# Amandaynzhou/MMT-PSM

Hardware: AMD Instinct MI355X
Metric: imgs/sec (student+teacher step, 1000x1000, AUG_K=2) (higher is better)
Workload: dtype f32

## Files before the change

### include/mmtpsm.h

```cpp
#ifndef MMTPSM_H
#define MMTPSM_H
#include <stdint.h>
#ifdef __cplusplus
extern "C" {
#endif

#define MMT_EINVAL (-22)

int mmt_version(void);

typedef struct {
  const float* feat[4];
  float* grad_feat[4];
  int H[4];
  int W[4];
  float scale[4];
  int num_levels;
  int N;
  int C;
} mmt_pyramid;

int mmt_roi_align_forward(const mmt_pyramid* pyr , const float* rois, const int32_t* levels,
                          int K, int PH, int PW, int sampling_ratio, float* out, void* stream);
int mmt_roi_align_forward_bf16(const mmt_pyramid* pyr , const float* rois, const int32_t* levels,
// ... 120 lines not shown
  int y_amax_stats;
  const void* f16_guard_x;
  const void* f16_guard_dy;
  const void* w_src;
  const void* w_src_scale;
  int x_planes_layout;
  void* y_rb;
  long y_rb_stride;
  const float* y_rb_scale;
  void* y_amax_next;
  int x_planes_lag;
  int y_rb_rows;
} mmt_conv_args;

int mmt_conv_forward(const mmt_conv_args* a , void* stream);
int mmt_conv_variant(const mmt_conv_args* a );
int mmt_conv_ksplit(const mmt_conv_args* a );
int mmt_conv_wants_planes(const mmt_conv_args* a );
int mmt_set_conv_precision(int mode);
int mmt_amax(const float* x, long n, const float* rowscale, long inner, int rows, float* amax , void* stream);
int mmt_amax_stats(const float* x, long n, float* slot , void* stream);
int mmt_sum_stats(const float* a, const float* b, const float* c, const float* d, float* y, long n,
                  float* slot , void* stream);
int mmt_stats_combine(const float* const* slots , int n, float* out , void* stream);
int mmt_split_planes_f16(const float* x, void* planes, long plane_stride, long n, float scale, const float* amax ,
                         float* scale_out , float* amax_next ,
                         float* zero_slot , void* stream);
int mmt_pack_weight_f16(const float* w, void* planes, long plane_stride, int Cout, int K, float scale, const float* amax,
                        float* scale_out, void* stream);
int mmt_pack_weight_flipped_f16(const float* w, const float* scale, void* planes, long plane_stride, int Cout, int KH, int KW,
                                int Cin, const float* amax, float* scale_out, void* stream);
int mmt_conv3x3_strip_f16x2(const mmt_conv_args* a , const float* s_x , const float* s_w , void* stream);
int mmt_conv_forward_f16x2(const mmt_conv_args* a , const float* x_amax , const float* s_w , void* stream);
int mmt_get_conv_precision(void);
int mmt_stem_fused(const float* x, int N, int H, int W, const float* w_s2d, const void* w_planes, long w_plane_stride,
                   const float* s_w , const float* scale, const float* shift, const float* x_slot , float* y,
                   float* y_slot , void* stream);
int mmt_c64_conv3_fused(const float* x, int N, int H, int W, const float* w2, const void* w2_planes, long w2_plane_stride,
                        const float* s_w2 , const float* scale2, const float* shift2, const float* x_slot ,
                        const float* w3, const void* w3_planes, long w3_plane_stride, const float* s_w3 , const float* scale3,
                        const float* shift3, const float* res, float* out, float* out_slot ,
                        const float* o2_scale , int o2_scale_is_amax, float* o2_amax_next ,
                        float* out_amax_next , const float* w1, const void* w1_planes, long w1_plane_stride,
                        const float* s_w1 , const float* scale1, const float* shift1, const float* out_scale ,
                        float* o1_next, float* o1_next_slot , void* stream);
int mmt_conv_wgrad_planes_splits(const mmt_conv_args* a );
int mmt_conv_wgrad_planes(const mmt_conv_args* a , const float* dy, const void* x_planes, long x_plane_stride,
                          const void* dy_planes, long dy_plane_stride, const float* s_x, const float* s_dy, const float* rowscale,
                          float* dw, float* dbias, float* workspace, void* stream);
typedef struct {
  void* fn;
  long a[16];
} mmt_call;
int mmt_replay(const mmt_call* calls , int n, int* failed_index );
int mmt_split_planes_f16_rb(const float* x, void* planes, long plane_stride, int rows, int W, int C, const float* amax,
                            float* scale_out, void* stream);
int mmt_conv_writes_rb(const mmt_conv_args* a );
typedef struct mmt_wgrad_job {
  mmt_conv_args a;
  const float* dy; const float* rowscale; float* dw; float* dbias;
  const void* x_planes; long x_plane_stride; const void* dy_planes; long dy_plane_stride; const float* s_x; const float* s_dy;
} mmt_wgrad_job;
int mmt_conv_wgrad_group_workspace(const mmt_wgrad_job* jobs , int n, long* floats_out );
int mmt_conv_wgrad_group(const mmt_wgrad_job* jobs , int n, float* workspace, long workspace_floats, void* stream);
int mmt_sum_stats_rb(const float* a, const float* b, const float* c, const float* d, float* y, int rows, int W, int C, float* slot,
                     void* planes, long plane_stride, const float* scale, float* amax_next, void* stream);
// ... 143 lines not shown
```

### mmt-psm_amd/csrc/conv_igemm.hip

```cpp
#include <stdlib.h>
#include <map>
#include <mutex>
#include <type_traits>
#include "conv_shared.h"

namespace {

template <int BM, int BN, int WM, int WN>
__device__ __forceinline__ void conv_epilogue_stage(f32x16 (&acc)[BM / (32 * WM)][BN / (32 * WN)], float* lds,
                                                    const int lane, const int wm, const int wn) {
  constexpr int TM = BM / (32 * WM), TN = BN / (32 * WN);
  float* ct = lds;
  const int col_l = lane & 31, rq = lane >> 5;
#pragma unroll
  for (int a = 0; a < TM; a++)
#pragma unroll
    for (int b = 0; b < TN; b++)
#pragma unroll
      for (int r = 0; r < 16; r++) {
        const int row = (wm * TM + a) * 32 + (r & 3) + 8 * (r >> 2) + 4 * rq;
        ct[row * BN + (wn * TN + b) * 32 + col_l] = acc[a][b][r];
      }
}


__device__ __forceinline__ void conv_amax_commit(const ConvP& p, AmaxAcc a, const int lin) {
  __shared__ float red[3][8];
  const int t = threadIdx.x, w = t >> 6, nw = (blockDim.x + 63) >> 6;
  const bool stats = p.amax_stats && (lin & 63) == 0;
#pragma unroll
  for (int o = 32; o > 0; o >>= 1) a.amx = fmaxf(a.amx, __shfl_xor(a.amx, o, 64));
  if (stats) {
#pragma unroll
    for (int o = 32; o > 0; o >>= 1) { a.asum += __shfl_xor(a.asum, o, 64); a.acnt += __shfl_xor(a.acnt, o, 64); }
  }
  if ((t & 63) == 0) { red[0][w] = a.amx; red[1][w] = a.asum; red[2][w] = a.acnt; }
  __syncthreads();
  if (t == 0) {
    float m = red[0][0], sm = red[1][0], cn = red[2][0];
    for (int i = 1; i < nw; i++) { m = fmaxf(m, red[0][i]); sm += red[1][i]; cn += red[2][i]; }
    const unsigned bits = __builtin_bit_cast(unsigned, m);
    if (m > 0.f && bits > __hip_atomic_load(p.amax_out, __ATOMIC_RELAXED, __HIP_MEMORY_SCOPE_AGENT)) atomicMax(p.amax_out, bits);
    if (p.amax_next && m > 0.f && bits > __hip_atomic_load(p.amax_next, __ATOMIC_RELAXED, __HIP_MEMORY_SCOPE_AGENT)) atomicMax(p.amax_next, bits);
    if (stats && cn > 0.f) {
      const int k = (lin >> 6) & 15;
      atomicAdd((float*)p.amax_out + 1 + k, sm);
      atomicAdd((float*)p.amax_out + 17 + k, cn);
    }
  }
}

template <int BM, int BN>
__device__ __forceinline__ void conv_epilogue_finish(const ConvP& p, float* lds, const int m0, const int n0, const int tid,
                                                     const int HoWo, AmaxAcc* acc = nullptr) {
  float amx = 0.f, asum = 0.f, acnt = 0.f;
  {
    float* ct = lds;
    constexpr int C4 = BN / 4, RPP = 256 / C4;
    const int cc = tid % C4, r0 = tid / C4;
    const int c = n0 + cc * 4;
    if (c < p.Cout) {
      const bool vec = (p.Cout & 3) == 0;
      const int nv = vec ? 4 : min(4, p.Cout - c);
      float sc[4], sh[4];
#pragma unroll
      for (int e = 0; e < 4; e++) {
        sc[e] = (p.scale && e < nv) ? p.scale[c + e] : 1.f;
        sh[e] = (p.shift && e < nv) ? p.shift[c + e] : 0.f;
      }
      auto ld = [&](const float* q, float* o) {
        if (vec) { const f32x4 t = ldg4(q); o[0] = t[0]; o[1] = t[1]; o[2] = t[2]; o[3] = t[3]; }
        else { for (int e = 0; e < 4; e++) o[e] = e < nv ? q[e] : 0.f; }
      };
      auto ldh = [&](const float* base, long idx, float* o) {
        const unsigned short* q = (const unsigned short*)base + idx;
        if (vec) {
          const uint2 t = *(const uint2*)q;
          o[0] = __builtin_bit_cast(float, t.x << 16); o[1] = __builtin_bit_cast(float, t.x & 0xffff0000u);
          o[2] = __builtin_bit_cast(float, t.y << 16); o[3] = __builtin_bit_cast(float, t.y & 0xffff0000u);
        } else { for (int e = 0; e < 4; e++) o[e] = e < nv ? __builtin_bit_cast(float, (unsigned)q[e] << 16) : 0.f; }
      };
      if (p.f16_sx) {
        const float inv = 1.f / ((p.f16_ax ? f16_scale_of(*p.f16_sx) : *p.f16_sx) * *p.f16_sw);
// ... 382 lines not shown
    const char* A = ring + buf * STAGE + (wm * TM * 32) * 32 + froff;
    const char* B = ring + buf * STAGE + NS * PA + (wn * TN * 32) * 32 + froff;
    bf16x8 fa[NS][TM], fb[NS][TN];
#pragma unroll
    for (int q = 0; q < NS; q++) {
#pragma unroll
      for (int a = 0; a < TM; a++) fa[q][a] = *(const bf16x8*)(A + q * PA + a * 32 * 32);
#pragma unroll
      for (int b = 0; b < TN; b++) fb[q][b] = *(const bf16x8*)(B + q * PB + b * 32 * 32);
    }
#pragma unroll
    for (int sum = 2 * (NS - 1) > NS - 1 ? NS - 1 : 0; sum >= 0; sum--)
#pragma unroll
      for (int qa = 0; qa <= sum; qa++) {
        const int qb = sum - qa;
        if (qa < NS && qb < NS) {
#pragma unroll
          for (int a = 0; a < TM; a++)
#pragma unroll
            for (int b = 0; b < TN; b++)
              acc[a][b] = __builtin_amdgcn_mfma_f32_32x32x16_bf16(fa[qa][a], fb[qb][b], acc[a][b], 0, 0, 0);
        }
      }
    if (kt + 1 < nkt) store_tile(buf ^ 1);
    __syncthreads();
  }
  conv_epilogue<BM, BN, WM, WN>(p, acc, lds, m0, n0, tid, lane, wm, wn, HoWo);
}

__device__ __attribute__((aligned(16))) const float g_zero16[4] = {0.f, 0.f, 0.f, 0.f};

__device__ __forceinline__ void dma16(const void* g, void* l) {
  __builtin_amdgcn_global_load_lds((const __attribute__((address_space(1))) void*)g, (lds_ptr_t)l, 16, 0, 0);
}

__device__ __forceinline__ void dma16_unseen(const void* g, void* l) {
#if defined(__HIP_DEVICE_COMPILE__)
  const unsigned la = __builtin_amdgcn_readfirstlane((unsigned)(unsigned long)(__attribute__((address_space(3))) char*)l);
  asm volatile("s_mov_b32 m0, %1\n\ts_nop 0\n\tglobal_load_lds_dwordx4 %0, off" ::"v"(g), "s"(la) : "m0", "memory");
#endif
}

template <int BM, int BN, int WM, int WN, int NS, int S, bool F16 = false>
__global__ __launch_bounds__(256, 2) void conv_fwd_glds_kernel(const ConvP p, const unsigned short* __restrict__ wpl,
                                                               const long wpl_stride, const int ksplit,
                                                               float* __restrict__ ws) {
  constexpr int TM = BM / (32 * WM), TN = BN / (32 * WN);
  constexpr int A_BYTES = BM * 64;
  constexpr int PB = BN * 32;
  constexpr int STAGE = A_BYTES + NS * PB;
  constexpr int NIA = BM / 64;
  constexpr int NIB_TOT = NS * BN / 32;
  constexpr int NIB = (NIB_TOT + 3) / 4;
  constexpr int NI = NIA + NIB;
  extern __shared__ __attribute__((aligned(16))) float lds[];
  char* const ring = (char*)lds;

  const int tid = threadIdx.x;
  const int lane = tid & 63;
  const int wave = __builtin_amdgcn_readfirstlane(tid >> 6);
  const int wm = wave / WN, wn = wave % WN;

  const int tiles_m = (p.M + BM - 1) / BM;
  const int tiles_n = (p.Cout + BN - 1) / BN;
  int bid = blockIdx.x;
  {
    const int nwg = tiles_m * tiles_n * ksplit, q = nwg >> 3, r = nwg & 7, xcd = bid & 7, idx = bid >> 3;
    bid = (xcd < r ? xcd * (q + 1) : r * (q + 1) + (xcd - r) * q) + idx;
  }
  const int ks = bid % ksplit;
  bid /= ksplit;
  const int tile_m = bid / tiles_n, tile_n = bid % tiles_n;
  const int m0 = tile_m * BM, n0 = tile_n * BN;
// ... 1492 lines not shown
```

### mmt-psm_amd/csrc/conv_shared.h

```cpp
#pragma once
#include <stdlib.h>
#include <type_traits>
#include "common.h"

namespace mmtconv {

struct ConvP {
  const float* x; const float* w; const float* scale; const float* shift; const float* res;
  const float* mask; const float* mul; float* y;
  int N, H, W, Cin, Cout, KH, KW, stride, pad, Ho, Wo;
  int relu, res_mode, out_stride, out_H, out_W;
  float mask_scale;
  int M, K, cin32, cin4;
  const unsigned short* wpl; long wpl_stride;
  const unsigned short* xpl; long xpl_stride;
  unsigned short* ypl; long ypl_stride;
  unsigned* amax_out;
  int amax_stats;
  int f16_ax;
  const float* f16_sx; const float* f16_sw;
  int io;
  const float* guard_x; const float* guard_dy;
  const float* w_src; const float* w_src_scale;
  int staged_epilogue;
// ... 64 lines not shown
  for (int q = 0; q < NS; q++) {
    const unsigned a = pk_bf16(r0, r1), b = pk_bf16(r2, r3);
    o[q] = uint2{a, b};
    if (q + 1 < NS) {
      r0 -= __builtin_bit_cast(float, a << 16);
      r1 -= __builtin_bit_cast(float, a & 0xffff0000u);
      r2 -= __builtin_bit_cast(float, b << 16);
      r3 -= __builtin_bit_cast(float, b & 0xffff0000u);
    }
  }
}
__device__ __forceinline__ float f16_scale_of(const float amax) {
  if (!(amax > 0.f)) return 1.f;
  int e;
  frexpf(amax, &e);
  e = 14 - e;
  e = e > 100 ? 100 : (e < -100 ? -100 : e);
  return ldexpf(1.f, e);
}

__device__ __forceinline__ f32x4 ldg4(const float* p) { return *(const f32x4*)p; }
__device__ __forceinline__ void split4h(const f32x4 v, const float s, uint2 (&o)[2]) {
  float r[4] = {v[0] * s, v[1] * s, v[2] * s, v[3] * s};
#pragma unroll
  for (int e = 0; e < 4; e++) r[e] = fminf(fmaxf(r[e], -65504.f), 65504.f);
  _Float16 h[4], l[4];
#pragma unroll
  for (int e = 0; e < 4; e++) { h[e] = (_Float16)r[e]; l[e] = (_Float16)(r[e] - (float)h[e]); }
  o[0] = uint2{__builtin_bit_cast(unsigned, f16x2{h[0], h[1]}), __builtin_bit_cast(unsigned, f16x2{h[2], h[3]})};
  o[1] = uint2{__builtin_bit_cast(unsigned, f16x2{l[0], l[1]}), __builtin_bit_cast(unsigned, f16x2{l[2], l[3]})};
}

struct AmaxAcc { float amx = 0.f, asum = 0.f, acnt = 0.f; };

__device__ __forceinline__ unsigned rb_split1(const float v, const float s) {
  const float r = __builtin_amdgcn_fmed3f(v * s, -65504.f, 65504.f);
  const _Float16 h = (_Float16)r;
  const _Float16 l = (_Float16)(r - (float)h);
  return __builtin_bit_cast(unsigned, f16x2{h, l});
}
struct RbGeom { int Wo; float rWo; unsigned cb32; };
__device__ __forceinline__ RbGeom rb_geom(const ConvP& p) {
  return RbGeom{p.Wo, 1.f / (float)p.Wo, (unsigned)(p.Cout >> 4) * (unsigned)p.Wo * 32u};
}
__device__ __forceinline__ unsigned rb_row_off(const RbGeom& g, const int m) {
  int row = (int)(((float)m + 0.5f) * g.rWo);
  int w = m - row * g.Wo;
  if (w < 0) { row--; w += g.Wo; } else if (w >= g.Wo) { row++; w -= g.Wo; }
  return (unsigned)row * g.cb32 + (unsigned)w * 32u;
}
__device__ __forceinline__ void rb_store4(const ConvP& p, const RbGeom& g, const int m, const int c, const f32x4 v, const float s) {
  uint2 o[2];
  split4h(v, s, o);
  char* const d = (char*)p.yrb + rb_row_off(g, m) + (unsigned)(c >> 4) * ((unsigned)g.Wo * 32u) + (unsigned)(c & 15) * 2u;
  *(uint2*)d = o[0];
  *(uint2*)(d + p.yrb_stride * 2) = o[1];
}
__device__ __forceinline__ void quad_transpose(unsigned (&w)[4], const int lane) {
  const bool o1 = lane & 1, o2 = lane & 2;
#pragma unroll
  for (int pr = 0; pr < 2; pr++) {
    const unsigned send = o1 ? w[2 * pr] : w[2 * pr + 1];
    const unsigned recv = (unsigned)__builtin_amdgcn_mov_dpp((int)send, 0xB1, 0xf, 0xf, true);
    if (o1) w[2 * pr] = recv; else w[2 * pr + 1] = recv;
  }
#pragma unroll
// ... 198 lines not shown
```

### mmt-psm_amd/maskrcnn_benchmark/_hip.py

```python
import ctypes
import weakref
import os
import threading as _threading

import torch

_HERE = os.path.dirname(os.path.abspath(__file__))
LIB_PATH = os.path.join(os.path.dirname(_HERE), "libmmtpsm.so")

c_void_p, c_int, c_float, c_double, c_int64 = ctypes.c_void_p, ctypes.c_int, ctypes.c_float, ctypes.c_double, ctypes.c_int64


class Pyramid(ctypes.Structure):
    _fields_ = [("feat", c_void_p * 4), ("grad_feat", c_void_p * 4), ("H", c_int * 4), ("W", c_int * 4),
                ("scale", c_float * 4), ("num_levels", c_int), ("N", c_int), ("C", c_int)]


class RoiMaps(ctypes.Structure):
    _fields_ = [("feat", c_void_p * 4), ("grad_feat", c_void_p * 4), ("H", c_int * 4), ("W", c_int * 4), ("C", c_int * 4),
                ("c_off", c_int * 4), ("scale", c_float * 4), ("num_maps", c_int), ("N", c_int), ("out_C", c_int)]


class ConvArgs(ctypes.Structure):
    _fields_ = [("x", c_void_p), ("w", c_void_p), ("scale", c_void_p), ("shift", c_void_p), ("res", c_void_p),
# ... 102 lines not shown
                            c_void_p, c_void_p, c_void_p, c_void_p, c_void_p],
    "mmt_position_embedding": [c_void_p, c_int, c_int, c_int, c_void_p, c_void_p, c_void_p],
    "mmt_sample_fg_bg_wide": [c_void_p, c_int, c_void_p, c_void_p, c_int, c_int, c_int, c_int, c_void_p, c_void_p, c_void_p, c_void_p,
                              c_void_p],
    "mmt_rpn_loss": [c_void_p, c_void_p, c_void_p, c_void_p, c_void_p, c_void_p, ctypes.c_long, c_float, c_void_p, c_void_p, c_void_p,
                     c_void_p, c_void_p],
    "mmt_box_loss": [c_void_p, c_void_p, c_void_p, c_void_p, c_int, c_int, c_void_p, c_void_p, c_void_p, c_void_p],
    "mmt_box_loss_rows": [c_void_p, c_void_p, c_void_p, c_void_p, c_int, c_int, c_void_p, c_void_p, c_void_p, c_void_p, c_void_p],
    "mmt_relation_attention_fwd": [c_void_p, c_void_p, c_void_p, c_void_p, c_void_p, c_int, c_int, c_int, c_int, c_int, c_int, c_float,
                                   c_void_p, c_void_p, c_void_p],
    "mmt_relation_attention_bwd": [c_void_p, c_void_p, c_void_p, c_void_p, c_void_p, c_void_p, c_int, c_int, c_int, c_int, c_int, c_float,
                                   c_void_p, c_void_p, c_void_p, c_void_p, c_void_p, c_void_p],
    "mmt_ciam_fwd": [c_void_p, c_void_p, c_int, c_int, c_int, c_int, c_void_p, c_void_p, c_void_p, c_void_p, c_void_p],
    "mmt_ciam_bwd": [c_void_p, c_void_p, c_int, c_int, c_int, c_int, c_void_p, c_void_p, c_void_p, c_void_p, c_void_p, c_void_p,
                     c_void_p, c_void_p, c_void_p],
    "mmt_stats_combine": [c_void_p, c_int, c_void_p, c_void_p],
    "mmt_sum_stats": [c_void_p, c_void_p, c_void_p, c_void_p, c_void_p, ctypes.c_long, c_void_p, c_void_p],
    "mmt_split_planes_f16": [c_void_p, c_void_p, ctypes.c_long, ctypes.c_long, c_float, c_void_p, c_void_p, c_void_p, c_void_p, c_void_p],
    "mmt_split_planes_f16_rb": [c_void_p, c_void_p, ctypes.c_long, c_int, c_int, c_int, c_void_p, c_void_p, c_void_p],
    "mmt_replay": [c_void_p, c_int, c_void_p],
    "mmt_conv_writes_rb": [ctypes.POINTER(ConvArgs)],
    "mmt_conv_wgrad_group_workspace": [c_void_p, c_int, ctypes.POINTER(ctypes.c_long)],
    "mmt_conv_wgrad_group": [c_void_p, c_int, c_void_p, ctypes.c_long, c_void_p],
    "mmt_sum_stats_rb": [c_void_p, c_void_p, c_void_p, c_void_p, c_void_p, c_int, c_int, c_int, c_void_p, c_void_p, ctypes.c_long, c_void_p,
                         c_void_p, c_void_p],
    "mmt_rb_scales_update": [c_void_p, c_int, c_void_p],
    "mmt_conv_wgrad_planes_splits": [ctypes.POINTER(ConvArgs)],
    "mmt_conv_wgrad_planes": [ctypes.POINTER(ConvArgs), c_void_p, c_void_p, ctypes.c_long, c_void_p, ctypes.c_long, c_void_p, c_void_p,
                              c_void_p, c_void_p, c_void_p, c_void_p, c_void_p],
    "mmt_pack_weight_f16": [c_void_p, c_void_p, ctypes.c_long, c_int, c_int, c_float, c_void_p, c_void_p, c_void_p],
    "mmt_pack_weight_flipped_f16": [c_void_p, c_void_p, c_void_p, ctypes.c_long, c_int, c_int, c_int, c_int, c_void_p, c_void_p, c_void_p],
    "mmt_conv3x3_strip_f16x2": [ctypes.POINTER(ConvArgs), c_void_p, c_void_p, c_void_p],
    "mmt_conv_forward_f16x2": [ctypes.POINTER(ConvArgs), c_void_p, c_void_p, c_void_p],
    "mmt_conv_forward_pg": [ctypes.POINTER(ConvArgs), c_void_p, c_void_p, c_int, c_int, c_void_p],
    "mmt_conv_pg_plan": [ctypes.POINTER(ConvArgs), c_void_p, c_void_p],
    "mmt_conv_pg_wanted": [ctypes.POINTER(ConvArgs)],
    "mmt_stem_fused": [c_void_p, c_int, c_int, c_int, c_void_p, c_void_p, ctypes.c_long, c_void_p, c_void_p, c_void_p, c_void_p, c_void_p,
                       c_void_p, c_void_p],
    "mmt_c64_conv3_fused": [c_void_p, c_int, c_int, c_int, c_void_p, c_void_p, ctypes.c_long, c_void_p, c_void_p, c_void_p, c_void_p, c_void_p,
                            c_void_p, ctypes.c_long, c_void_p, c_void_p, c_void_p, c_void_p, c_void_p, c_void_p, c_void_p, c_int, c_void_p,
                            c_void_p, c_void_p, c_void_p, ctypes.c_long, c_void_p, c_void_p, c_void_p, c_void_p, c_void_p, c_void_p,
                            c_void_p],
    "mmt_maxpool3x3s2_bf16": [c_void_p, c_void_p, c_int, c_int, c_int, c_int, c_int, c_int, c_void_p],
    "mmt_gconv3x3_forward": [c_void_p, c_void_p, c_void_p, c_void_p, c_void_p, c_int, c_int, c_int, c_int, c_int, c_int, c_int, c_void_p],
    "mmt_gconv3x3_dgrad": [c_void_p, c_void_p, c_void_p, c_void_p, c_void_p, c_void_p, c_int, c_int, c_int, c_int, c_int, c_int, c_void_p],
    "mmt_gconv3x3_wgrad": [c_void_p, c_void_p, c_void_p, c_void_p, c_int, c_int, c_int, c_int, c_int, c_int, c_void_p],
    "mmt_maxpool3x3s2_backward": [c_void_p, c_void_p, c_void_p, c_int, c_int, c_int, c_int, c_void_p],
    "mmt_stem_wgrad": [c_void_p, c_void_p, c_void_p, c_void_p, c_int, c_int, c_int, c_void_p],
    "mmt_mask_bce": [c_void_p, c_void_p, c_void_p, c_int, c_int, c_int, c_float, c_void_p, c_void_p, c_void_p],
    "mmt_mgd_level_forward": [c_void_p, ctypes.POINTER(MgdTeachers), c_void_p, c_int, c_int, c_int, c_int, c_void_p, c_void_p],
    "mmt_mgd_level_backward": [c_void_p, ctypes.POINTER(MgdTeachers), c_void_p, c_int, c_int, c_int, c_int, c_void_p, c_void_p, c_void_p],
    "mmt_mgd_views_forward": [ctypes.POINTER(MgdStudents), ctypes.POINTER(MgdTeachers), c_void_p, c_int, c_int, c_int, c_int, c_void_p,
                              c_void_p],
    "mmt_mgd_views_backward": [ctypes.POINTER(MgdStudents), ctypes.POINTER(MgdTeachers), c_void_p, c_int, c_int, c_int, c_int, c_void_p,
                               c_void_p, c_void_p],
    "mmt_mask_pool": [c_void_p, c_int, c_int, c_int, c_int, c_int, c_void_p, c_void_p],
    "mmt_psm_rows": [c_void_p, c_int, c_void_p, c_int, c_int, c_void_p, c_float, c_int, c_int, c_void_p, c_void_p, c_void_p],
    "mmt_psm_variance": [c_void_p, c_int, c_int, c_int, c_int, c_void_p, c_void_p],
    "mmt_ema_update": [c_void_p, c_void_p, c_int64, c_double, c_void_p],
    "mmt_sgd_momentum": [c_void_p, c_void_p, c_void_p, c_int64, c_float, c_float, c_float, c_int, c_void_p],
    "mmt_grad_guard": [c_void_p, c_int64, c_void_p, c_void_p, c_float, c_void_p],
    "mmt_sgd_momentum_guarded": [c_void_p, c_void_p, c_void_p, c_int64, c_float, c_float, c_float, c_int, c_void_p, c_void_p],
    "mmt_paste_masks": [c_void_p, c_void_p, c_void_p, c_void_p, c_int, c_int, c_int, c_int, c_int, c_float, c_void_p, c_void_p],
    "mmt_paste_mask_stack": [c_void_p, c_void_p, c_int, c_int, c_int, c_int, c_float, c_void_p, c_void_p],
    "mmt_polygon_targets": [c_void_p, c_void_p, c_void_p, c_void_p, c_int, c_int, c_void_p, c_void_p, c_void_p],
    "mmt_mask_pack": [c_void_p, c_int, c_int, c_int, c_void_p, c_void_p, c_void_p],
# ... 422 lines not shown
    if not PG_RB:
        xp, st = f16_split(x)
        return xp, st, 0, 0
    rb = _rb_of(x)
    if rb is not None and rb[3] == "epi" and (rb[4] is None or rb[4] >= x.shape[0]):
        F16_STATS["rb_epi"] = F16_STATS.get("rb_epi", 0) + 1
        return rb[0], rb[1], 1, 1
    F16_STATS["rb_split"] = F16_STATS.get("rb_split", 0) + 1
    N, C, Hh, W = x.shape
    if x.numel() >= (1 << 30) or C % 16:
        xp, st = f16_split(x)
        return xp, st, 0, 0
    am = _amax_of(x)
    xp = torch.empty((2, x.numel()), dtype=torch.float16, device=x.device)
    st = torch.empty((1,), dtype=torch.float32, device=x.device)
    _check(lib().mmt_split_planes_f16_rb(x.data_ptr(), xp.data_ptr(), xp.stride(0), N * Hh, W, C, am[0].data_ptr(), st.data_ptr(), _stream()),
           "mmt_split_planes_f16_rb")
    _rb_attach(x, xp, st, "split")
    return xp, st, 1, 0


def _pack_f16(w, scale, flipped, pl, am):
    Cout, Cin, KH, KW = w.shape
    F16_STATS["weight_pack"] = F16_STATS.get("weight_pack", 0) + 1
    _check(lib().mmt_amax(w.data_ptr(), w.numel(), _p(scale) if flipped else None, Cin * KH * KW, Cout, am.data_ptr(), _stream()), "mmt_amax")
    if flipped:
        _check(lib().mmt_pack_weight_flipped_f16(w.data_ptr(), _p(scale), pl.data_ptr(), pl.stride(0), Cout, KH, KW, Cin,
                                                 am.data_ptr(), am.data_ptr() + 4, _stream()), "mmt_pack_weight_flipped_f16")
    else:
        _check(lib().mmt_pack_weight_f16(w.data_ptr(), pl.data_ptr(), pl.stride(0), Cout, Cin * KH * KW, 1.0, am.data_ptr(),
                                         am.data_ptr() + 4, _stream()), "mmt_pack_weight_f16")


def f16_weight_planes(w, flip_scale=None, flipped=False):
    form = "f16_dgrad" if flipped else "f16"
    flat, hit = _flat_form(w, form, flip_scale)
    if hit is not None:
        return hit
    stamp = _loose_stamp(w, flip_scale, w)
    hit = LOOSE.get(w, form, stamp, flip_scale)
    if hit is not None:
        return hit
    Cout, Cin, KH, KW = w.shape
    am = torch.zeros((2,), dtype=torch.float32, device=w.device)
    pl = torch.empty((2, packed_elems(Cin, KH * KW * Cout) if flipped else packed_elems(Cout, Cin * KH * KW)), dtype=torch.float16,
                     device=w.device)
    _pack_f16(w, flip_scale, flipped, pl, am)
    if flipped and flat is not None and flat.register(form, w, flip_scale, pl, am):
        return pl, am[1:2]
    return LOOSE.put(w, form, stamp, flip_scale, (pl, am[1:2]), w, am)


def set_bf16_storage(on):
    global _BF16_STORAGE
    if on and _DET:
        raise NotImplementedError("bf16 activation storage is not offered in deterministic mode (its kernels' summation orders were "
                                  "never examined): set_deterministic(False)")
    _BF16_STORAGE = bool(on)


def bf16_storage():
    return _BF16_STORAGE and get_conv_precision() == 1


_DET = os.environ.get("MMT_DETERMINISTIC", "0") != "0"
_DET_TORCH = None
COLSUM_MAX_BLOCKS, MASK_BCE_WS, MGD_MAX_BLOCKS, RPN_LOSS_MAX_BLOCKS, BOX_LOSS_MAX_BLOCKS = 256, 2048, 4096, 1024, 256


def _det_torch(on):
    global _DET_TORCH
    from torch.utils import deterministic as td
    if on:
        if _DET_TORCH is None:
            _DET_TORCH = (torch.are_deterministic_algorithms_enabled(), torch.is_deterministic_algorithms_warn_only_enabled(),
                          td.fill_uninitialized_memory)
        torch.use_deterministic_algorithms(True)
        td.fill_uninitialized_memory = False
    elif _DET_TORCH is not None:
        torch.use_deterministic_algorithms(_DET_TORCH[0], warn_only=_DET_TORCH[1])
        td.fill_uninitialized_memory = _DET_TORCH[2]
        _DET_TORCH = None

# ... 1042 lines not shown
    if planes_owner is not None:
        planes_owner.ensure_bf16()
    _check(lib().mmt_conv_forward(ctypes.byref(a), _stream()), "mmt_conv_forward")
    if rec:
        _profiled(a, e0, "fwd%d" % var, lib().mmt_conv_ksplit(ctypes.byref(a)), pre, ebytes)
    if y_planes is not None:
        y._mmt_planes = (y_planes, y._version)
    if amax_slot is not None:
        y._mmt_amax = (amax_slot, y._version)
    return y


def conv_forward_pg(x, w, scale=None, shift=None, stride=1, pad=0, relu=False, res=None, mask=None, mask_scale=1.0, w_shape=None,
                    f16_src=None, tile_rows=0, ksplit=0, xp=None):
    x = nhwc(x)
    N, Cin, H, W = x.shape
    src = (nhwc(w), False, None) if w is not None else (nhwc(f16_src[0]), True, f16_src[1])
    Cout, KH, KW = _weight_dims(Cin, src[0].shape if w is not None else w_shape)
    Ho, Wo = _conv_out_hw(H, W, KH, KW, stride, pad)
    a = _conv_shape(ConvArgs(), N, H, W, Cin, Cout, KH, KW, stride, pad, Ho, Wo)
    a.x = x.data_ptr()
    y = empty_nhwc(N, Cout, Ho, Wo, x.device)
    a.y = y.data_ptr()
    a.scale, a.shift, a.relu = _p(scale), _p(shift), 1 if relu else 0
    if res is not None:
        a.res, a.res_mode = nhwc(res).data_ptr(), 1
    if mask is not None:
        a.mask, a.mask_scale = nhwc(mask).data_ptr(), float(mask_scale)
    slot = _amax_slot(x.device)
    a.y_amax, a.y_amax_stats = slot.ptr, 1
    return _conv_f16(a, K_PG, x, src, y, slot, None, int(tile_rows), int(ksplit), xp, None, False)


def stem_fused(x, w_s2d, scale, shift):
    _dev(x)
    N, C, Hh, W = x.shape
    if C != 3 or not x.is_contiguous() or x.dtype != torch.float32 or (Hh & 3) or (W & 3) or tuple(w_s2d.shape) != (64, 16, 4, 4):
        raise RuntimeError("stem_fused: (N, 3, H, W) fp32 NCHW with H, W % 4 == 0 and the 64 x 16 x 4 x 4 space-to-depth filter")
    w = nhwc(w_s2d)
    am = _amax_of(x)
    if type(am[0]) is not _Slot:
        raise RuntimeError("stem_fused: the input needs a full statistics slot")
    wp16, sw = f16_weight_planes(w)
    y = empty_nhwc(N, 64, Hh // 4, W // 4, x.device)
    slot = _amax_slot(x.device)
    _check(lib().mmt_stem_fused(x.data_ptr(), N, Hh, W, w.data_ptr(), wp16.data_ptr(), wp16.stride(0), sw.data_ptr(), _p(scale), _p(shift),
                                am[0].ptr, y.data_ptr(), slot.ptr, _stream()), "mmt_stem_fused")
    y._mmt_amax = (slot, y._version)
    return y


C64_FUSE = os.environ.get("MMT_C64_FUSE", "1") != "0"


def o2_site(w3):
    return ("o2", w3.data_ptr())


def c64_fuse_enabled():
    return bool(C64_FUSE and F16X2 and RB_EPI and PROFILE is None and os.environ.get("MMT_C64") != "0" and get_conv_precision() == 3)


def out_site(w1_next):
    return ("out1", w1_next.data_ptr())


# ... 1047 lines not shown
```

### mmt-psm_amd/maskrcnn_benchmark/layers/fused.py

```python
import torch

from .. import _hip as H


_NONE = {}


def _none_like(x):
    t = _NONE.get(x.device)
    if t is None:
        t = _NONE[x.device] = torch.empty((0,), dtype=torch.float32, device=x.device)
    return t


def _dst(t):
    return getattr(t, "_flat_grad", None) if t is not None else None


def _touch(*slots):
    for d in slots:
        if d is not None:
            ent = H.GRAD_SLOTS.get(d.data_ptr())
            if ent is not None and ent[0]() is not None:
                ent[0]().touched.add(ent[1])
# ... 400 lines not shown
    @staticmethod
    def backward(ctx, g2, g3, g4, g5):
        sv = ctx.saved_tensors
        cs, inner, wi, wl = sv[0:4], sv[4:8], sv[8:12], sv[12:16]
        gs = [g2, g3, g4, g5]
        gs = [H.nhwc(g) if g is not None else torch.zeros_like(inner[k]) for k, g in enumerate(gs)]
        d_in = [None] * 4
        dwl, dbl, dwi, dbi, dcs = [None] * 4, [None] * 4, [None] * 4, [None] * 4, [None] * 4
        for k in range(4):
            d_in[k] = _dgrad(gs[k], wl[k], inner[k].shape, 1, 1, None, res=d_in[k - 1] if k > 0 else None,
                             res_mode=3 if k > 0 else 0)
            dwl[k], dbl[k] = _wgrad(inner[k], gs[k], wl[k], 1, 1, None, True, *ctx.dst[1][k])
        for k in range(4):
            dwi[k], dbi[k] = _wgrad(cs[k], d_in[k], wi[k], 1, 0, None, True, *ctx.dst[0][k])
            if ctx.needs_input_grad[k]:
                dcs[k] = _dgrad(d_in[k], wi[k], cs[k].shape, 1, 0, None, mask=cs[k], out_dtype=cs[k].dtype)
        out = list(dcs)
        for k in range(4):
            out += [dwi[k], dbi[k]]
        for k in range(4):
            out += [dwl[k], dbl[k]]
        return tuple(out) + (None, None)


class DeconvFn(torch.autograd.Function):

    @staticmethod
    def forward(ctx, x, w, b, relu, input_relu):
        x = H.nhwc(x)
        w_in = w
        w = H.nhwc(w)
        P, Cin, h, wd_ = x.shape
        Cout = w.shape[1]
        y = H.empty_nhwc(P, Cout, 2 * h, 2 * wd_, x.device)
        wf = w.permute(2, 3, 1, 0).contiguous()
        for kh in range(2):
            for kw in range(2):
                H.conv_forward(x, wf[kh, kw].view(Cout, Cin, 1, 1), None, b, relu=relu, out_stride=2,
                               out_hw=(2 * h, 2 * wd_), y_out=y, y_offset=(kh * 2 * wd_ + kw) * Cout)
        ctx.save_for_backward(x, w)
        ctx.cfgv = (input_relu, b is not None)
        ctx.dst = (_dst(w_in), _dst(b))
        return y

    @staticmethod
    def backward(ctx, g):
        x, w = ctx.saved_tensors
        input_relu, has_b = ctx.cfgv
        g = H.nhwc(g)
        dx = dw = db = None
        if ctx.needs_input_grad[1]:
            dst_w, dst_b = ctx.dst
            dw = dst_w if dst_w is not None else torch.zeros_like(w)
            H.conv_wgrad(g, x, tuple(w.shape), 2, 0, dw)
            _touch(dst_w, dst_b if has_b else None)
            if has_b:
                db = dst_b if dst_b is not None else torch.zeros((w.shape[1],), dtype=torch.float32, device=w.device)
                H.colsum(g, db)
                db = None if dst_b is not None else db
            dw = None if dst_w is not None else dw
        if ctx.needs_input_grad[0]:
            dx = H.conv_forward(g, w, stride=2, pad=0, mask=x if input_relu else None, rb_site=("dx", w.data_ptr()))
        return dx, dw, db, None, None


class RoiAlignFpnFn(torch.autograd.Function):

    @staticmethod
    def forward(ctx, rois, levels, res, scales, sr, *feats):
        feats = [H.nhwc(f) for f in feats]
        out = H.roi_align_forward(feats, scales, rois, levels, res, res, sr)
        if out.dtype == torch.float32 and H.F16X2 and H.get_conv_precision() == 3:
# ... 193 lines not shown


def relu_grad_mask(x):
    return ReluGradMaskFn.apply(x) if x.requires_grad else x


class SplitBatchFn(torch.autograd.Function):

    @staticmethod
    def forward(ctx, x, n):
        ctx.n, ctx.shape = n, x.shape
        return x[:n], x[n:]

    @staticmethod
    def backward(ctx, ga, gb):
        n, shape = ctx.n, ctx.shape
        out = H.empty_nhwc(shape[0], shape[1], shape[2], shape[3], (ga if ga is not None else gb).device)
        if ga is not None:
            out[:n].copy_(ga)
        else:
            out[:n].zero_()
        if gb is not None:
            out[n:].copy_(gb)
        else:
            out[n:].zero_()
        return out, None


def split_batch(x, n):
    return SplitBatchFn.apply(x, n)


_FORK_ON = True


_FORK_ACC = _os.environ.get("MMT_FORK_ACC", "1") != "0"


class _ForkAcc(object):
    __slots__ = ("buf", "fresh", "seen", "rb_site")

    def __init__(self, rb_site):
        self.buf, self.fresh, self.seen, self.rb_site = None, False, [], rb_site

    def put(self, t, fresh):
        first = self.buf is None
        if t is not self.buf:
            self.seen.append(t)
        self.buf, self.fresh = t, fresh
        if not fresh:
            H.drop(t)
        return first


class ForkFn(torch.autograd.Function):

    @staticmethod
    def forward(ctx, x, n, rb_site=None, acc=None):
        ctx.set_materialize_grads(False)
        ctx.rb_site = rb_site
        ctx.acc = acc
        return tuple(x.view_as(x) for _ in range(n))

    @staticmethod
    def backward(ctx, *gs):
        gs = [g for g in gs if g is not None]
# ... 78 lines not shown
```

Before: 135.4.

## Fuse 2x2 deconv forward into one f16x2 MFMA kernel launch

Adds a dedicated HIP kernel that computes all four taps of the 2x2 transposed convolution as a single GEMM over Cout*4 columns. It uses split-f16 MFMA, streams the weights into LDS through double-buffered DMA, and scatters results directly into the strided output. This replaces four separate conv_forward launches plus a per-call weight permute/contiguous copy, and reuses the activation load across all taps. Unsupported shapes or precisions fall back to the old path, and a slow scalar fallback runs when the guard flags bad inputs. Shared helpers move into conv_shared.h.

```diff
diff --git a/include/mmtpsm.h b/include/mmtpsm.h
--- a/include/mmtpsm.h
+++ b/include/mmtpsm.h
@@ -176,6 +176,7 @@
                                 int Cin, const float* amax, float* scale_out, void* stream);
 int mmt_conv3x3_strip_f16x2(const mmt_conv_args* a , const float* s_x , const float* s_w , void* stream);
 int mmt_conv_forward_f16x2(const mmt_conv_args* a , const float* x_amax , const float* s_w , void* stream);
+int mmt_deconv2x2_forward_f16x2(const mmt_conv_args* a , const float* x_amax , const float* s_w , void* stream);
 int mmt_get_conv_precision(void);
 int mmt_stem_fused(const float* x, int N, int H, int W, const float* w_s2d, const void* w_planes, long w_plane_stride,
                    const float* s_w , const float* scale, const float* shift, const float* x_slot , float* y,
diff --git a/mmt-psm_amd/csrc/conv_igemm.hip b/mmt-psm_amd/csrc/conv_igemm.hip
--- a/mmt-psm_amd/csrc/conv_igemm.hip
+++ b/mmt-psm_amd/csrc/conv_igemm.hip
@@ -23,32 +23,6 @@
       }
 }
 
-
-__device__ __forceinline__ void conv_amax_commit(const ConvP& p, AmaxAcc a, const int lin) {
-  __shared__ float red[3][8];
-  const int t = threadIdx.x, w = t >> 6, nw = (blockDim.x + 63) >> 6;
-  const bool stats = p.amax_stats && (lin & 63) == 0;
-#pragma unroll
-  for (int o = 32; o > 0; o >>= 1) a.amx = fmaxf(a.amx, __shfl_xor(a.amx, o, 64));
-  if (stats) {
-#pragma unroll
-    for (int o = 32; o > 0; o >>= 1) { a.asum += __shfl_xor(a.asum, o, 64); a.acnt += __shfl_xor(a.acnt, o, 64); }
-  }
-  if ((t & 63) == 0) { red[0][w] = a.amx; red[1][w] = a.asum; red[2][w] = a.acnt; }
-  __syncthreads();
-  if (t == 0) {
-    float m = red[0][0], sm = red[1][0], cn = red[2][0];
-    for (int i = 1; i < nw; i++) { m = fmaxf(m, red[0][i]); sm += red[1][i]; cn += red[2][i]; }
-    const unsigned bits = __builtin_bit_cast(unsigned, m);
-    if (m > 0.f && bits > __hip_atomic_load(p.amax_out, __ATOMIC_RELAXED, __HIP_MEMORY_SCOPE_AGENT)) atomicMax(p.amax_out, bits);
-    if (p.amax_next && m > 0.f && bits > __hip_atomic_load(p.amax_next, __ATOMIC_RELAXED, __HIP_MEMORY_SCOPE_AGENT)) atomicMax(p.amax_next, bits);
-    if (stats && cn > 0.f) {
-      const int k = (lin >> 6) & 15;
-      atomicAdd((float*)p.amax_out + 1 + k, sm);
-      atomicAdd((float*)p.amax_out + 17 + k, cn);
-    }
-  }
-}
 
 template <int BM, int BN>
 __device__ __forceinline__ void conv_epilogue_finish(const ConvP& p, float* lds, const int m0, const int n0, const int tid,
@@ -497,13 +471,6 @@
 
 __device__ __forceinline__ void dma16(const void* g, void* l) {
   __builtin_amdgcn_global_load_lds((const __attribute__((address_space(1))) void*)g, (lds_ptr_t)l, 16, 0, 0);
-}
-
-__device__ __forceinline__ void dma16_unseen(const void* g, void* l) {
-#if defined(__HIP_DEVICE_COMPILE__)
-  const unsigned la = __builtin_amdgcn_readfirstlane((unsigned)(unsigned long)(__attribute__((address_space(3))) char*)l);
-  asm volatile("s_mov_b32 m0, %1\n\ts_nop 0\n\tglobal_load_lds_dwordx4 %0, off" ::"v"(g), "s"(la) : "m0", "memory");
-#endif
 }
 
 template <int BM, int BN, int WM, int WN, int NS, int S, bool F16 = false>
diff --git a/mmt-psm_amd/csrc/conv_shared.h b/mmt-psm_amd/csrc/conv_shared.h
--- a/mmt-psm_amd/csrc/conv_shared.h
+++ b/mmt-psm_amd/csrc/conv_shared.h
@@ -120,6 +120,39 @@
 }
 
 struct AmaxAcc { float amx = 0.f, asum = 0.f, acnt = 0.f; };
+
+__device__ __forceinline__ void conv_amax_commit(const ConvP& p, AmaxAcc a, const int lin) {
+  __shared__ float red[3][8];
+  const int t = threadIdx.x, w = t >> 6, nw = (blockDim.x + 63) >> 6;
+  const bool stats = p.amax_stats && (lin & 63) == 0;
+#pragma unroll
+  for (int o = 32; o > 0; o >>= 1) a.amx = fmaxf(a.amx, __shfl_xor(a.amx, o, 64));
+  if (stats) {
+#pragma unroll
+    for (int o = 32; o > 0; o >>= 1) { a.asum += __shfl_xor(a.asum, o, 64); a.acnt += __shfl_xor(a.acnt, o, 64); }
+  }
+  if ((t & 63) == 0) { red[0][w] = a.amx; red[1][w] = a.asum; red[2][w] = a.acnt; }
+  __syncthreads();
+  if (t == 0) {
+    float m = red[0][0], sm = red[1][0], cn = red[2][0];
+    for (int i = 1; i < nw; i++) { m = fmaxf(m, red[0][i]); sm += red[1][i]; cn += red[2][i]; }
+    const unsigned bits = __builtin_bit_cast(unsigned, m);
+    if (m > 0.f && bits > __hip_atomic_load(p.amax_out, __ATOMIC_RELAXED, __HIP_MEMORY_SCOPE_AGENT)) atomicMax(p.amax_out, bits);
+    if (p.amax_next && m > 0.f && bits > __hip_atomic_load(p.amax_next, __ATOMIC_RELAXED, __HIP_MEMORY_SCOPE_AGENT)) atomicMax(p.amax_next, bits);
+    if (stats && cn > 0.f) {
+      const int k = (lin >> 6) & 15;
+      atomicAdd((float*)p.amax_out + 1 + k, sm);
+      atomicAdd((float*)p.amax_out + 17 + k, cn);
+    }
+  }
+}
+
+__device__ __forceinline__ void dma16_unseen(const void* g, void* l) {
+#if defined(__HIP_DEVICE_COMPILE__)
+  const unsigned la = __builtin_amdgcn_readfirstlane((unsigned)(unsigned long)(__attribute__((address_space(3))) char*)l);
+  asm volatile("s_mov_b32 m0, %1\n\ts_nop 0\n\tglobal_load_lds_dwordx4 %0, off" ::"v"(g), "s"(la) : "m0", "memory");
+#endif
+}
 
 __device__ __forceinline__ unsigned rb_split1(const float v, const float s) {
   const float r = __builtin_amdgcn_fmed3f(v * s, -65504.f, 65504.f);
diff --git a/mmt-psm_amd/csrc/deconv.hip b/mmt-psm_amd/csrc/deconv.hip
--- /dev/null
+++ b/mmt-psm_amd/csrc/deconv.hip
@@ -0,0 +1,222 @@
+#include <atomic>
+#include "conv_shared.h"
+
+namespace {
+
+__device__ __noinline__ void deconv_slow_block(const ConvPK pk, const int m0, const int n_lo, const int n_hi, const int lin) {
+  const int C = pk->Cout >> 2, HW = pk->H * pk->W, ncols = n_hi - n_lo;
+  float amx = 0.f, asum = 0.f, acnt = 0.f;
+  for (int o = threadIdx.x; o < 128 * ncols; o += blockDim.x) {
+    const int i = o / ncols, n = n_lo + (o - i * ncols);
+    const int m = m0 + i;
+    if (m >= pk->M) break;
+    const int img = m / HW, rem = m - img * HW;
+    const int h = rem / pk->W, w = rem - h * pk->W;
+    const float* xr = pk->x + (long)m * pk->Cin;
+    const float* wr = pk->w_src + n;
+    float acc = 0.f;
+    for (int ci = 0; ci < pk->Cin; ci++) acc = fmaf(xr[ci], wr[(long)ci * pk->Cout], acc);
+    const int tap = n / C, co = n - tap * C;
+    float v = acc + (pk->shift ? pk->shift[co] : 0.f);
+    if (pk->relu) v = fmaxf(v, 0.f);
+    pk->y[(((long)img * pk->out_H + 2 * h + (tap >> 1)) * pk->out_W + 2 * w + (tap & 1)) * C + co] = v;
+    const float av = fabsf(v);
+    amx = fmaxf(amx, av); asum += av; acnt += 1.f;
+  }
+  if (pk->amax_out) {
+    if (amx > 0.f) atomicMax(pk->amax_out, __builtin_bit_cast(unsigned, amx));
+    if (pk->amax_stats && (lin & 63) == 0 && acnt > 0.f) {
+      const int k = (lin >> 6) & 15;
+      atomicAdd((float*)pk->amax_out + 1 + k, asum);
+      atomicAdd((float*)pk->amax_out + 17 + k, acnt);
+    }
+  }
+}
+
+template <int KT>
+__global__ __launch_bounds__(256, 2) void deconv2x2_rows_kernel(const ConvP p, const unsigned short* __restrict__ wpl,
+                                                                const long wpl_stride, const int ppb) {
+  constexpr int NS = 2, BN = 32;
+  constexpr int PIECES = KT * NS;
+  constexpr int BBUF = PIECES * 1024;
+  constexpr unsigned OOB = 0x80000000u;
+  static_assert(PIECES % 4 == 0, "pieces per wave");
+  extern __shared__ __attribute__((aligned(16))) float lds[];
+  char* const bring = (char*)lds;
+  unsigned* const rowb = (unsigned*)(bring + 2 * BBUF);
+  float* const shl = (float*)(bring + 2 * BBUF + 512);
+  const int tid = threadIdx.x, lane = tid & 63;
+  const int wave = __builtin_amdgcn_readfirstlane(tid >> 6);
+  const int lr = lane & 31, kh2 = lane >> 5;
+  const int m0 = blockIdx.x * 128;
+  const int K = 16 * KT;
+  const int C = p.Cout >> 2;
+  const int nb32 = p.Cout >> 5, ptap = C >> 5;
+  const int nt_lo = blockIdx.y * ppb, nt_hi = min(nb32, nt_lo + ppb);
+  const int cnt = nt_hi - nt_lo;
+  if (cnt <= 0) return;
+  const F16Guard guard = f16_guard_load(p.guard_x);
+  auto issue_b = [&](int nt, int buf) {
+#pragma unroll
+    for (int i = 0; i < PIECES / 4; i++) {
+      const int piece = wave + 4 * i;
+      const int kt = piece / NS, q = piece % NS;
+      dma16_unseen(wpl + q * wpl_stride + ((long)kt * nb32 + nt) * 512 + lane * 8, bring + buf * BBUF + piece * 1024);
+    }
+  };
+  const int rot = blockIdx.x % cnt;
+  auto pn = [&](int i) {
+    int t = i + rot;
+    if (t >= cnt) t -= cnt;
+    return nt_lo + t;
+  };
+  issue_b(pn(0), 0);
+  if (f16_guard_bad(guard)) {
+    asm volatile("s_waitcnt vmcnt(0)" ::: "memory");
+    deconv_slow_block(kernarg_convp(), m0, nt_lo * BN, nt_hi * BN, blockIdx.x + gridDim.x * blockIdx.y);
+    return;
+  }
+  if (tid < 128) {
+    const int m = m0 + tid;
+    unsigned b = OOB;
+    if (m < p.M) {
+      const int HW = p.H * p.W;
+      const int img = m / HW, rem = m - img * HW;
+      const int h = rem / p.W, w = rem - h * p.W;
+      b = (unsigned)((img * p.out_H + 2 * h) * p.out_W + 2 * w) * ((unsigned)C * 4u);
+    }
+    rowb[tid] = b;
+  }
+  for (int c = tid; c < C; c += 256) shl[c] = p.shift ? p.shift[c] : 0.f;
+  uint4 fa[KT][NS];
+  const float sx = f16_scale_of(*p.f16_sx);
+  const float finv = 1.f / (sx * *p.f16_sw);
+  const int boff = lr * 32 + (((kh2 ^ (lr >> 3)) & 1) << 4);
+  const int col_l = lane & 31, rq = lane >> 5;
+  const __amdgpu_buffer_rsrc_t ry = __builtin_amdgcn_make_buffer_rsrc((void*)p.y, 0, (int)((long)p.M * p.Cout * 4), 0x00020000);
+  {
+    const __amdgpu_buffer_rsrc_t rsrc = __builtin_amdgcn_make_buffer_rsrc((void*)p.x, 0, (int)((long)p.M * K * 4), 0x00020000);
+    const int m = m0 + wave * 32 + lr;
+    const unsigned base = m < p.M ? ((unsigned)m * (unsigned)K + 8u * kh2) * 4u : OOB;
+    constexpr int CH = KT < 8 ? KT : 8;
+#pragma unroll
+    for (int k0 = 0; k0 < KT; k0 += CH) {
+      f32x4 ra[CH][2];
+#pragma unroll
+      for (int kt = 0; kt < CH; kt++)
+#pragma unroll
+        for (int h = 0; h < 2; h++)
+          ra[kt][h] = __builtin_bit_cast(f32x4, __builtin_amdgcn_raw_buffer_load_b128(rsrc, (int)(base + (k0 + kt) * 64 + h * 16), 0, 0));
+#pragma unroll
+      for (int kt = 0; kt < CH; kt++) {
+        uint2 o0[NS], o1[NS];
+        split4h(ra[kt][0], sx, o0);
+        split4h(ra[kt][1], sx, o1);
+#pragma unroll
+        for (int q = 0; q < NS; q++) fa[k0 + kt][q] = uint4{o0[q].x, o0[q].y, o1[q].x, o1[q].y};
+      }
+      if (KT > CH) __builtin_amdgcn_sched_barrier(0);
+    }
+  }
+  asm volatile("s_waitcnt vmcnt(0)" ::: "memory");
+  __syncthreads();
+  unsigned yb[16];
+#pragma unroll
+  for (int r = 0; r < 16; r++) yb[r] = rowb[wave * 32 + 4 * rq + 8 * (r >> 2) + (r & 3)];
+  float amx = 0.f, asum = 0.f, acnt = 0.f;
+  for (int i = 0; i < cnt; i++) {
+    const int buf = i & 1;
+    __syncthreads();
+    asm volatile("" ::: "memory");
+    if (i + 1 < cnt) issue_b(pn(i + 1), buf ^ 1);
+    asm volatile("" ::: "memory");
+    const int nt = pn(i);
+    const int tap = nt / ptap, co0 = (nt - tap * ptap) * BN;
+    const float sh = shl[co0 + col_l];
+    f32x16 acc;
+#pragma unroll
+    for (int r = 0; r < 16; r++) acc[r] = 0.f;
+    const char* bb = bring + buf * BBUF + boff;
+    uint4 fb[2][NS];
+    auto read_b = [&](int kt, uint4 (&f)[NS]) {
+#pragma unroll
+      for (int q = 0; q < NS; q++) f[q] = *(const uint4*)(bb + (kt * NS + q) * 1024);
+    };
+    read_b(0, fb[0]);
+#pragma unroll
+    for (int kt = 0; kt < KT; kt++) {
+      if (kt + 1 < KT) read_b(kt + 1, fb[(kt + 1) & 1]);
+      acc = __builtin_amdgcn_mfma_f32_32x32x16_f16(__builtin_bit_cast(f16x8, fa[kt][0]), __builtin_bit_cast(f16x8, fb[kt & 1][1]), acc, 0, 0, 0);
+      acc = __builtin_amdgcn_mfma_f32_32x32x16_f16(__builtin_bit_cast(f16x8, fa[kt][1]), __builtin_bit_cast(f16x8, fb[kt & 1][0]), acc, 0, 0, 0);
+      acc = __builtin_amdgcn_mfma_f32_32x32x16_f16(__builtin_bit_cast(f16x8, fa[kt][0]), __builtin_bit_cast(f16x8, fb[kt & 1][0]), acc, 0, 0, 0);
+      __builtin_amdgcn_sched_barrier(0);
+    }
+    const unsigned toff = ((unsigned)((tap >> 1) * p.out_W + (tap & 1)) * (unsigned)C + (unsigned)(co0 + col_l)) * 4u;
+#pragma unroll
+    for (int r = 0; r < 16; r++) {
+      float v = acc[r] * finv + sh;
+      v = p.relu ? fmaxf(v, 0.f) : v;
+      const bool ok = yb[r] != OOB;
+      const float av = ok ? fabsf(v) : 0.f;
+      amx = fmaxf(amx, av);
+      asum += av;
+      acnt += ok ? 1.f : 0.f;
+      __builtin_amdgcn_raw_buffer_store_b32(__builtin_bit_cast(unsigned, v), ry, (int)(yb[r] + toff), 0, 0);
+    }
+    asm volatile("s_waitcnt vmcnt(0)" ::: "memory");
+  }
+  if (p.amax_out) conv_amax_commit(p, AmaxAcc{amx, asum, acnt}, blockIdx.y * gridDim.x + blockIdx.x);
+}
+
+template <int KT>
+int launch_deconv(const ConvP& p, hipStream_t s) {
+  const size_t lds = 2 * (size_t)KT * 2 * 1024 + 512 + (size_t)p.Cout;
+  auto kern = deconv2x2_rows_kernel<KT>;
+  constexpr size_t lds_max = 2 * (size_t)KT * 2 * 1024 + 512 + 8192;
+  if (lds_max > 65536) {
+    static std::atomic<unsigned long long> done{0};
+    int dev = 0;
+    if (hipGetDevice(&dev) != hipSuccess) return MMT_EINVAL;
+    const unsigned long long bit = 1ull << (dev & 63);
+    if (dev >= 64 || !(done.load(std::memory_order_acquire) & bit)) {
+      const hipError_t e = hipFuncSetAttribute((const void*)kern, hipFuncAttributeMaxDynamicSharedMemorySize, (int)lds_max);
+      if (e != hipSuccess) return (int)e;
+      if (dev < 64) done.fetch_or(bit, std::memory_order_release);
+    }
+  }
+  const int tiles_m = mmt_cdiv(p.M, 128), npanel = p.Cout >> 5;
+  int groups = 1;
+  long best = -1;
+  for (int g = 1; g <= npanel && g <= 16; g++) {
+    const long cost = (long)mmt_cdiv((long)tiles_m * g, 512) * (mmt_cdiv(npanel, g) + 4);
+    if (best < 0 || cost < best) { best = cost; groups = g; }
+  }
+  const int ppb = mmt_cdiv(npanel, groups);
+  hipLaunchKernelGGL(kern, dim3(tiles_m, mmt_cdiv(npanel, ppb)), dim3(256), lds, s, p, p.wpl, p.wpl_stride, ppb);
+  MMT_LAUNCH_CHECK();
+  return 0;
+}
+
+}
+
+extern "C" int mmt_deconv2x2_forward_f16x2(const mmt_conv_args* a, const float* x_amax, const float* s_w, void* stream) {
+  ConvP p;
+  const int e = fill(p, a);
+  if (e) return e;
+  if (!p.y || !p.wpl || !p.w_src || !x_amax || !s_w) return MMT_EINVAL;
+  if (p.io || p.ypl || p.xpl || p.xpl_rb || p.yrb || p.amax_next || p.res || p.res_mode || p.mask || p.mul || p.scale) return MMT_EINVAL;
+  if (p.KH != 1 || p.KW != 1 || p.stride != 1 || p.pad != 0 || p.Ho != p.H || p.Wo != p.W || p.out_stride != 2 ||
+      p.out_H != 2 * p.H || p.out_W != 2 * p.W)
+    return MMT_EINVAL;
+  if ((p.Cin != 64 && p.Cin != 128 && p.Cin != 256) || p.Cout <= 0 || (p.Cout & 127) || p.Cout > 8192) return MMT_EINVAL;
+  if (((size_t)p.x & 15) || ((size_t)p.y & 3) || ((size_t)p.wpl & 15) || (p.wpl_stride & 7) ||
+      p.wpl_stride < (long)(p.Cin >> 4) * (p.Cout >> 5) * 512)
+    return MMT_EINVAL;
+  if ((long)p.M * p.Cout * 4 >= (1L << 31) || (long)p.M * p.Cin * 4 >= (1L << 31)) return MMT_EINVAL;
+  if (p.M == 0) return 0;
+  p.f16_sx = x_amax; p.f16_sw = s_w; p.f16_ax = 1;
+  hipStream_t s = (hipStream_t)stream;
+  if (p.Cin == 64) return launch_deconv<4>(p, s);
+  if (p.Cin == 128) return launch_deconv<8>(p, s);
+  return launch_deconv<16>(p, s);
+}
diff --git a/mmt-psm_amd/maskrcnn_benchmark/_hip.py b/mmt-psm_amd/maskrcnn_benchmark/_hip.py
--- a/mmt-psm_amd/maskrcnn_benchmark/_hip.py
+++ b/mmt-psm_amd/maskrcnn_benchmark/_hip.py
@@ -158,6 +158,7 @@
     "mmt_pack_weight_flipped_f16": [c_void_p, c_void_p, c_void_p, ctypes.c_long, c_int, c_int, c_int, c_int, c_void_p, c_void_p, c_void_p],
     "mmt_conv3x3_strip_f16x2": [ctypes.POINTER(ConvArgs), c_void_p, c_void_p, c_void_p],
     "mmt_conv_forward_f16x2": [ctypes.POINTER(ConvArgs), c_void_p, c_void_p, c_void_p],
+    "mmt_deconv2x2_forward_f16x2": [ctypes.POINTER(ConvArgs), c_void_p, c_void_p, c_void_p],
     "mmt_conv_forward_pg": [ctypes.POINTER(ConvArgs), c_void_p, c_void_p, c_int, c_int, c_void_p],
     "mmt_conv_pg_plan": [ctypes.POINTER(ConvArgs), c_void_p, c_void_p],
     "mmt_conv_pg_wanted": [ctypes.POINTER(ConvArgs)],
@@ -646,13 +647,14 @@
                                          am.data_ptr() + 4, _stream()), "mmt_pack_weight_f16")
 
 
-def f16_weight_planes(w, flip_scale=None, flipped=False):
+def f16_weight_planes(w, flip_scale=None, flipped=False, owner=None):
     form = "f16_dgrad" if flipped else "f16"
     flat, hit = _flat_form(w, form, flip_scale)
     if hit is not None:
         return hit
-    stamp = _loose_stamp(w, flip_scale, w)
-    hit = LOOSE.get(w, form, stamp, flip_scale)
+    owner = w if owner is None else owner
+    stamp = _loose_stamp(w, flip_scale, owner)
+    hit = LOOSE.get(owner, form, stamp, flip_scale)
     if hit is not None:
         return hit
     Cout, Cin, KH, KW = w.shape
@@ -662,7 +664,7 @@
     _pack_f16(w, flip_scale, flipped, pl, am)
     if flipped and flat is not None and flat.register(form, w, flip_scale, pl, am):
         return pl, am[1:2]
-    return LOOSE.put(w, form, stamp, flip_scale, (pl, am[1:2]), w, am)
+    return LOOSE.put(owner, form, stamp, flip_scale, (pl, am[1:2]), w, am)
 
 
 def set_bf16_storage(on):
@@ -1771,6 +1773,41 @@
     return _conv_f16(a, K_PG, x, src, y, slot, None, int(tile_rows), int(ksplit), xp, None, False)
 
 
+def deconv2x2_forward(x, w, shift=None, relu=False):
+    if not (F16X2 and get_conv_precision() == 3 and not _BF16_STORAGE and x.dtype == torch.float32 and w.dtype == torch.float32):
+        return None
+    P, Cin, h, wd = x.shape
+    C = w.shape[1]
+    if (P == 0 or h == 0 or wd == 0 or Cin not in (64, 128, 256) or C == 0 or C % 32 or C > 2048 or tuple(w.shape) != (Cin, C, 2, 2)
+            or P * h * wd * 16 * C >= (1 << 31) or P * h * wd * 4 * Cin >= (1 << 31) or x.data_ptr() % 16):
+        return None
+    if shift is not None and (shift.dtype != torch.float32 or not shift.is_contiguous() or shift.numel() != C):
+        return None
+    am = _recorded(x)
+    if am is None:
+        return None
+    view = w.permute(0, 2, 3, 1).reshape(Cin, 4 * C, 1, 1)
+    if view.data_ptr() != w.data_ptr() or not _site_ok((w.data_ptr(), "deconv"), x):
+        return None
+    a = _conv_shape(ConvArgs(), P, h, wd, Cin, 4 * C, 1, 1, 1, 0, h, wd)
+    a.out_stride, a.out_H, a.out_W = 2, 2 * h, 2 * wd
+    y = empty_nhwc(P, C, 2 * h, 2 * wd, x.device)
+    a.x, a.y, a.shift, a.relu = x.data_ptr(), y.data_ptr(), _p(shift), 1 if relu else 0
+    a.w_src = w.data_ptr()
+    a.f16_guard_x = _guard(am)
+    wp16, sw = f16_weight_planes(view, None, True, owner=w)
+    a.w_planes, a.w_plane_stride = wp16.data_ptr(), wp16.stride(0)
+    slot = _amax_slot(x.device)
+    a.y_amax, a.y_amax_stats = slot.ptr, 1
+    F16_STATS["deconv"] = F16_STATS.get("deconv", 0) + 1
+    e0 = _ev() if PROFILE is not None else None
+    _check(lib().mmt_deconv2x2_forward_f16x2(ctypes.byref(a), am[0].data_ptr(), sw.data_ptr(), _stream()), "mmt_deconv2x2_forward_f16x2")
+    if e0 is not None:
+        PROFILE.append((2.0 * P * h * wd * 4 * C * Cin, e0, _ev(), ("fwd3", P, h, wd, Cin, 4 * C, 1, 1, 1), 1, None, 0))
+    y._mmt_amax = (slot, y._version)
+    return y
+
+
 def stem_fused(x, w_s2d, scale, shift):
     _dev(x)
     N, C, Hh, W = x.shape
diff --git a/mmt-psm_amd/maskrcnn_benchmark/layers/fused.py b/mmt-psm_amd/maskrcnn_benchmark/layers/fused.py
--- a/mmt-psm_amd/maskrcnn_benchmark/layers/fused.py
+++ b/mmt-psm_amd/maskrcnn_benchmark/layers/fused.py
@@ -456,12 +456,14 @@
         w = H.nhwc(w)
         P, Cin, h, wd_ = x.shape
         Cout = w.shape[1]
-        y = H.empty_nhwc(P, Cout, 2 * h, 2 * wd_, x.device)
-        wf = w.permute(2, 3, 1, 0).contiguous()
-        for kh in range(2):
-            for kw in range(2):
-                H.conv_forward(x, wf[kh, kw].view(Cout, Cin, 1, 1), None, b, relu=relu, out_stride=2,
-                               out_hw=(2 * h, 2 * wd_), y_out=y, y_offset=(kh * 2 * wd_ + kw) * Cout)
+        y = H.deconv2x2_forward(x, w, b, relu) if _DECONV_ONE_LAUNCH and not H.get_deterministic() else None
+        if y is None:
+            y = H.empty_nhwc(P, Cout, 2 * h, 2 * wd_, x.device)
+            wf = w.permute(2, 3, 1, 0).contiguous()
+            for kh in range(2):
+                for kw in range(2):
+                    H.conv_forward(x, wf[kh, kw].view(Cout, Cin, 1, 1), None, b, relu=relu, out_stride=2,
+                                   out_hw=(2 * h, 2 * wd_), y_out=y, y_offset=(kh * 2 * wd_ + kw) * Cout)
         ctx.save_for_backward(x, w)
         ctx.cfgv = (input_relu, b is not None)
         ctx.dst = (_dst(w_in), _dst(b))
@@ -721,6 +723,7 @@
 
 
 _FORK_ON = True
+_DECONV_ONE_LAUNCH = True
 
 
 _FORK_ACC = _os.environ.get("MMT_FORK_ACC", "1") != "0"
```

After: 135.9, median of 2. About the same (+0.4%).
